# Zhiyu014/GNN-UDS

Measured on AMD Instinct MI355X. Metric: graph-steps/sec (forward rollout), |V|=10k |E|=12k d=64, higher is better.
Workload: dtype f32 storage/accumulate, GEMM operands as bf16 hi+lo split (3 MFMA products)

## Files before the change

gnn_uds_amd/csrc/kernels_fused_ws.hpp:

```cpp
#pragma once
#include "kernels_fused.hpp"

namespace uds {

constexpr int WS_NY = 4, WS_NX = FUSED_WAVES - WS_NY;
constexpr int WS_XPRIO = 1;
constexpr int WS_OCT_WD = 4;
constexpr int WS_OCT_GRP = 1;

inline int64_t fused_ws_lds_bytes(int p_cap, int q_cap, int meta_cap) {
  return 4 * ((int64_t)meta_cap + 4 * p_cap + 3 * FUSED_D + FUSED_H + 2 * (int64_t)q_cap * SEC_STRIDE + 2 * (int64_t)p_cap * FUSED_D);
}

template <int IMM>
__device__ __forceinline__ void ws_gld16(f32x4 &dst, const float *base, unsigned voff) {
  asm volatile("global_load_dwordx4 %0, %1, %2 offset:%3" : "=v"(dst) : "v"(voff), "s"(base), "n"(IMM) : "memory");
}
__device__ __forceinline__ void ws_pin4(f32x4 &a0, f32x4 &a1, f32x4 &a2, f32x4 &a3) {
  asm volatile("" : "+v"(a0), "+v"(a1), "+v"(a2), "+v"(a3));
}
__device__ __forceinline__ void row8_max4(const float (&in)[4], float (&out)[4]) {
  asm("s_nop 1\n\t" UDS_DPP4_FIRST("v_max_f32_dpp", "quad_perm:[1,0,3,2]") UDS_DPP4("v_max_f32_dpp", "quad_perm:[2,3,0,1]")
      UDS_DPP4("v_max_f32_dpp", "row_half_mirror")
      : "=&v"(out[0]), "=&v"(out[1]), "=&v"(out[2]), "=&v"(out[3])
      : "v"(in[0]), "v"(in[1]), "v"(in[2]), "v"(in[3]));
}
__device__ __forceinline__ void row8_sum4(const float (&in)[4], float (&out)[4]) {
  asm("s_nop 1\n\t" UDS_DPP4_FIRST("v_add_f32_dpp", "quad_perm:[1,0,3,2]") UDS_DPP4("v_add_f32_dpp", "quad_perm:[2,3,0,1]")
      UDS_DPP4("v_add_f32_dpp", "row_half_mirror")
      : "=&v"(out[0]), "=&v"(out[1]), "=&v"(out[2]), "=&v"(out[3])
      : "v"(in[0]), "v"(in[1]), "v"(in[2]), "v"(in[3]));
}
template <int HI>
__device__ __forceinline__ unsigned ws_add_half(unsigned pk, unsigned base) {
  unsigned r;
  if (HI) asm("v_add_u32_sdwa %0, %1, %2 dst_sel:DWORD dst_unused:UNUSED_PAD src0_sel:WORD_1 src1_sel:DWORD" : "=v"(r) : "v"(pk), "v"(base));
  else asm("v_add_u32_sdwa %0, %1, %2 dst_sel:DWORD dst_unused:UNUSED_PAD src0_sel:WORD_0 src1_sel:DWORD" : "=v"(r) : "v"(pk), "v"(base));
  return r;
}
__device__ __forceinline__ void ws_vmcnt(int n) {
  switch (n) {
    case 0: asm volatile("s_waitcnt vmcnt(0)" ::: "memory"); break;
    case 1: asm volatile("s_waitcnt vmcnt(1)" ::: "memory"); break;
    case 2: asm volatile("s_waitcnt vmcnt(2)" ::: "memory"); break;
    case 3: asm volatile("s_waitcnt vmcnt(3)" ::: "memory"); break;
    case 4: asm volatile("s_waitcnt vmcnt(4)" ::: "memory"); break;
    case 5: asm volatile("s_waitcnt vmcnt(5)" ::: "memory"); break;
    case 6: asm volatile("s_waitcnt vmcnt(6)" ::: "memory"); break;
    case 7: asm volatile("s_waitcnt vmcnt(7)" ::: "memory"); break;
    default: asm volatile("s_waitcnt vmcnt(8)" ::: "memory"); break;
  }
}

template <int ACT>
__global__ __launch_bounds__(FUSED_WAVES * 64, 2) void k_fused_ws(FusedArgs a) {
  constexpr int NT = FUSED_WAVES * 64, NY = WS_NY, NX = WS_NX;
  constexpr int FP = 64, FS = 64;
  constexpr int U = FUSED_U;
  extern __shared__ __attribute__((aligned(16))) int32_t smem[];

  const int tid = threadIdx.x, lane = tid & 63;
  const int wave = __builtin_amdgcn_readfirstlane(tid >> 6);
  const bool team_y = wave < NY;
  const int yw = wave, xw = wave - NY;

  const int W = gridDim.x, b = blockIdx.x;
  const int q8 = W / 8, r8 = W % 8, xcd = b % 8;
  const int w = (xcd < r8 ? xcd * (q8 + 1) : r8 * (q8 + 1) + (xcd - r8) * q8) + b / 8;
  const int tile = w % a.n_tiles;
  const int chunk_id = w / a.n_tiles;
  const int s_begin = chunk_id * a.chunk;
  const int s_end = min(a.S, (chunk_id + 1) * a.chunk);
  const int sd = __builtin_amdgcn_readfirstlane(a.hdr[tile * TILE_HDR_INTS + 6]);
  if (!((a.side_mask >> sd) & 1)) return;
  const FusedSide &S_ = a.side[sd];

  float *s_self = reinterpret_cast<float *>(smem + a.meta_cap);
  float *s_nbr = s_self + 2 * a.p_cap;
  float *attn = s_nbr + 2 * a.p_cap;
  float *sec = attn + 3 * FUSED_D + FUSED_H;
  float *hx = sec + 2 * a.q_cap * SEC_STRIDE;
  const int sec_buf = a.q_cap * SEC_STRIDE, hx_buf = a.p_cap * FUSED_D;

  {
    const uint4 *src = reinterpret_cast<const uint4 *>(a.blocks + (int64_t)tile * a.meta_cap);
    uint4 *dst = reinterpret_cast<uint4 *>(smem);
    for (int i = tid; i < a.meta_cap / 4; i += NT) dst[i] = src[i];
  }
  if (tid < FUSED_D) {
    attn[tid] = S_.a_self[tid] * 1.44269504088896340736f;
    attn[FUSED_D + tid] = S_.a_nbr[tid] * 1.44269504088896340736f;
    if (tid < FUSED_H) attn[2 * FUSED_D + tid] = S_.b_small ? S_.b_small[tid] : 0.f;
    attn[2 * FUSED_D + FUSED_H + tid] = S_.b_out ? S_.b_out[tid] : 0.f;
  }
  __syncthreads();
  const int n_own = __builtin_amdgcn_readfirstlane(smem[0]), n_prim = __builtin_amdgcn_readfirstlane(smem[1]),
            n_sec = __builtin_amdgcn_readfirstlane(smem[2]), flags = __builtin_amdgcn_readfirstlane(smem[3]),
            n_ovf = __builtin_amdgcn_readfirstlane(smem[4]), n_adj = __builtin_amdgcn_readfirstlane(smem[5]),
            inc_width = __builtin_amdgcn_readfirstlane(smem[7]);
  const EllOffsets off = ell_offsets(n_own, n_prim, n_sec, flags, n_ovf, n_adj);
  const int32_t *prim_ids = smem + off.prim;
  const int32_t *sec_ids = smem + off.sec;
  const uint32_t *inc_loc = reinterpret_cast<const uint32_t *>(smem + off.inc_loc);
  int32_t *inc_w = smem + off.inc_w;
  const f32x4 *inc_val4 = reinterpret_cast<const f32x4 *>(inc_w);
  const unsigned char *adj_b = reinterpret_cast<const unsigned char *>(smem + off.adj);
  const int32_t *ovf_ptr = smem + off.ovf_ptr, *ovf_loc = smem + off.ovf_loc;
  int32_t *ovf_w = smem + off.ovf_w;
  const int32_t *adj_ptr = smem + off.adj_ptr, *adj_loc = smem + off.adj_loc;

  for (int i = tid; i < ELL_INC * n_prim; i += NT) {
    const int k = inc_w[i];
    reinterpret_cast<float *>(inc_w)[i] = k >= 0 ? S_.ne_val[k] : 0.f;
  }
  if (flags & ELL_FLAG_INC_OVF)
    for (int i = tid; i < n_ovf; i += NT) reinterpret_cast<float *>(ovf_w)[i] = S_.ne_val[ovf_w[i]];
  const float *ovf_val = reinterpret_cast<const float *>(ovf_w);

#ifdef UDS_PHASE_TIMING
  unsigned long long tm_[8] = {0, 0, 0, 0, 0, 0, 0, 0}, tl_ = clock64();
  const unsigned long long rt0_ = __builtin_amdgcn_s_memrealtime(), mt0_ = tl_;
#define WS_STAMP(k) do { const unsigned long long n_ = clock64(); tm_[k] += n_ - tl_; tl_ = n_; } while (0)
#define WS_DUMP() do { if (a.dbg && lane == 0) { unsigned long long *o = a.dbg + ((size_t)blockIdx.x * 8 + wave) * 16; \
    for (int q_ = 0; q_ < 7; ++q_) o[q_] = tm_[q_]; o[12] = wave; \
    o[15] = ((__builtin_amdgcn_s_memrealtime() - rt0_) << 32) | ((clock64() - mt0_) & 0xffffffffull); \
    o[7] = 1ull | ((unsigned long long)sd << 8) | ((unsigned long long)n_own << 16) | ((unsigned long long)n_prim << 32) | ((unsigned long long)n_sec << 48); } } while (0)
#else
#define WS_STAMP(k) do { } while (0)
#define WS_DUMP() do { } while (0)
#endif
  const int64_t sec_stride = (int64_t)S_.n_sec_glob * FS, prim_stride = (int64_t)S_.n_prim_glob * FP;
  const int n_snap = s_end - s_begin;

  __syncthreads();
  if (team_y) {
    typedef float f32x16 __attribute__((ext_vector_type(16)));
    constexpr int KT32 = (FP + FUSED_H) / 16, KX32 = FP / 16, MB32 = FUSED_D / 32;
    static_assert(NY == 4, "one 32-row block per Y wave: four waves cover p_cap = 128");
    const int n32 = lane & 31, hf = lane >> 5;
    bf16x8 wh[KT32][MB32], wl[KT32][MB32];
#pragma unroll
    for (int t = 0; t < KT32; ++t)
#pragma unroll
      for (int m = 0; m < MB32; ++m) {
        wh[t][m] = __builtin_bit_cast(bf16x8, S_.w_big32[((t * MB32 + m) * 2 + 0) * 64 + lane]);
        wl[t][m] = __builtin_bit_cast(bf16x8, S_.w_big32[((t * MB32 + m) * 2 + 1) * 64 + lane]);
      }
    const int lrow = 32 * yw + n32;
    const bool valid = lrow < n_prim;
    const int lr = min(lrow, n_prim - 1);
    const unsigned prow = (unsigned)prim_ids[lr] * FP + 8u * hf;
    f32x4 pp[2 * KX32];
    const bool has_rem = S_.rem != nullptr;
    const unsigned rrow = (unsigned)prim_ids[lr] * FUSED_H + 8u * hf;
    f32x4 rm[4] = {f32x4{0.f, 0.f, 0.f, 0.f}, f32x4{0.f, 0.f, 0.f, 0.f}, f32x4{0.f, 0.f, 0.f, 0.f}, f32x4{0.f, 0.f, 0.f, 0.f}};
    const int64_t rem_stride = (int64_t)S_.n_prim_glob * FUSED_H;
    const unsigned ag_locs = inc_loc[lr];
    const f32x4 ag_vals = inc_val4[lr];
    __builtin_amdgcn_s_waitcnt(0x0F70);
    if (n_snap > 0) {
      const float *base = S_.prim_in + s_begin * prim_stride;
      static_for<2 * KX32>([&](auto i_) {
        constexpr int i = decltype(i_)::value;
        pp[i] = *reinterpret_cast<const f32x4 *>(base + prow + 16 * (i >> 1) + 4 * (i & 1));
      });
      if (has_rem) {
        const float *rb = S_.rem + s_begin * rem_stride + rrow;
        rm[0] = *reinterpret_cast<const f32x4 *>(rb);
        rm[1] = *reinterpret_cast<const f32x4 *>(rb + 4);
        rm[2] = *reinterpret_cast<const f32x4 *>(rb + 16);
        rm[3] = *reinterpret_cast<const f32x4 *>(rb + 20);
      }
    }
    WS_STAMP(0);
    lds_barrier();

    auto mfma3_32 = [&](const bf16x8 &a_h, const bf16x8 &a_l, const bf16x8 &d_h, const bf16x8 &d_l, f32x16 acc) __attribute__((always_inline)) {
      acc = __builtin_amdgcn_mfma_f32_32x32x16_bf16(a_h, d_l, acc, 0, 0, 0);
      acc = __builtin_amdgcn_mfma_f32_32x32x16_bf16(a_l, d_h, acc, 0, 0, 0);
      acc = __builtin_amdgcn_mfma_f32_32x32x16_bf16(a_h, d_h, acc, 0, 0, 0);
      return acc;
    };
    for (int k = 0; k <= n_snap; ++k) {
      if (k < n_snap && 32 * yw < n_prim) {
        const bool more = k + 1 < n_snap;
        const float *next = S_.prim_in + (s_begin + k + 1) * prim_stride;
        const float *secr = sec + (k & 1) * sec_buf;
        float *hxw = hx + (k & 1) * hx_buf;
        float *ssw = s_self + (k & 1) * a.p_cap, *snw = s_nbr + (k & 1) * a.p_cap;
        bf16x8 dh[KT32], dl[KT32];
        static_for<KX32>([&](auto t_) {
          constexpr int t = decltype(t_)::value;
          const f32x4 u0 = pp[2 * t], u1 = pp[2 * t + 1];
          split8(make_float4(u0[0], u0[1], u0[2], u0[3]), make_float4(u1[0], u1[1], u1[2], u1[3]), dh[t], dl[t]);
        });
        if (more)
          static_for<2 * KX32>([&](auto i_) {
            constexpr int i = decltype(i_)::value;
            pp[i] = *reinterpret_cast<const f32x4 *>(next + prow + 16 * (i >> 1) + 4 * (i & 1));
          });
        f32x16 acc[MB32];
#pragma unroll
        for (int m = 0; m < MB32; ++m)
#pragma unroll
          for (int r = 0; r < 16; ++r) acc[m][r] = 0.f;
#pragma unroll
        for (int t = 0; t < KX32; ++t)
#pragma unroll
          for (int m = 0; m < MB32; ++m) acc[m] = mfma3_32(wh[t][m], wl[t][m], dh[t], dl[t], acc[m]);
        float4 g0 = make_float4(rm[0][0], rm[0][1], rm[0][2], rm[0][3]), g1 = make_float4(rm[1][0], rm[1][1], rm[1][2], rm[1][3]),
               g2 = make_float4(rm[2][0], rm[2][1], rm[2][2], rm[2][3]), g3 = make_float4(rm[3][0], rm[3][1], rm[3][2], rm[3][3]);
        if (more && has_rem) {
          const float *rb = S_.rem + (s_begin + k + 1) * rem_stride + rrow;
          rm[0] = *reinterpret_cast<const f32x4 *>(rb);
          rm[1] = *reinterpret_cast<const f32x4 *>(rb + 4);
          rm[2] = *reinterpret_cast<const f32x4 *>(rb + 16);
          rm[3] = *reinterpret_cast<const f32x4 *>(rb + 20);
        }
        auto fma4 = [&](float4 &g, float wv, const float4 &u) { g.x = fmaf(wv, u.x, g.x); g.y = fmaf(wv, u.y, g.y); g.z = fmaf(wv, u.z, g.z); g.w = fmaf(wv, u.w, g.w); };
        auto add_row = [&](unsigned la, float wa) {
          const float *ra = secr + la * SEC_STRIDE + 8 * hf;
          const float4 u0 = *reinterpret_cast<const float4 *>(ra), u1 = *reinterpret_cast<const float4 *>(ra + 4);
          const float4 u2 = *reinterpret_cast<const float4 *>(ra + 16), u3 = *reinterpret_cast<const float4 *>(ra + 20);
          fma4(g0, wa, u0); fma4(g1, wa, u1); fma4(g2, wa, u2); fma4(g3, wa, u3);
        };
        add_row(ag_locs & 0xffu, ag_vals[0]);
        add_row((ag_locs >> 8) & 0xffu, ag_vals[1]);
        if (inc_width > 2) {
          add_row((ag_locs >> 16) & 0xffu, ag_vals[2]);
          add_row(ag_locs >> 24, ag_vals[3]);
        }
        if (flags & ELL_FLAG_INC_OVF)
          for (int p = ovf_ptr[lr]; p < ovf_ptr[lr + 1]; ++p) add_row((unsigned)ovf_loc[p], ovf_val[p]);
        split8(g0, g1, dh[KX32], dl[KX32]);
        split8(g2, g3, dh[KX32 + 1], dl[KX32 + 1]);
#pragma unroll
        for (int t = KX32; t < KT32; ++t)
#pragma unroll
          for (int m = 0; m < MB32; ++m) acc[m] = mfma3_32(wh[t][m], wl[t][m], dh[t], dl[t], acc[m]);
        float ps = 0.f, pn = 0.f;
#pragma unroll
        for (int m = 0; m < MB32; ++m)
#pragma unroll
          for (int gq = 0; gq < 4; ++gq) {
            const f32x4 as4 = *reinterpret_cast<const f32x4 *>(attn + 32 * m + 8 * gq + 4 * hf);
            const f32x4 an4 = *reinterpret_cast<const f32x4 *>(attn + FUSED_D + 32 * m + 8 * gq + 4 * hf);
#pragma unroll
            for (int q = 0; q < 4; ++q) {
              ps = fmaf(acc[m][4 * gq + q], as4[q], ps);
              pn = fmaf(acc[m][4 * gq + q], an4[q], pn);
            }
          }
        ps += __shfl_xor(ps, 32);
        pn += __shfl_xor(pn, 32);
        if (valid) {
          if (hf == 0) {
            ssw[lrow] = ps;
            snw[lrow] = pn;
          }
#pragma unroll
          for (int m = 0; m < MB32; ++m)
#pragma unroll
            for (int gq = 0; gq < 4; ++gq) {
              const f32x4 o = {acc[m][4 * gq], acc[m][4 * gq + 1], acc[m][4 * gq + 2], acc[m][4 * gq + 3]};
              *reinterpret_cast<f32x4 *>(hxw + lrow * FUSED_D + (((8 * m + 2 * gq + hf) ^ (lrow & 7)) << 2)) = o;
            }
        }
      }
      WS_STAMP(1);
      lds_barrier();
      WS_STAMP(2);
    }
    WS_DUMP();
  } else {
    __builtin_amdgcn_s_setprio(WS_XPRIO);
    typedef float f32x16 __attribute__((ext_vector_type(16)));
    constexpr int KS32 = FS / 16, SJ32 = (8 + NX - 1) / NX;
    const int n32 = lane & 31, hf = lane >> 5;
    bf16x8 w1h[KS32], w1l[KS32];
#pragma unroll
    for (int t = 0; t < KS32; ++t) {
      w1h[t] = __builtin_bit_cast(bf16x8, S_.w_small32[(t * 2 + 0) * 64 + lane]);
      w1l[t] = __builtin_bit_cast(bf16x8, S_.w_small32[(t * 2 + 1) * 64 + lane]);
    }
    unsigned srow[SJ32];
#pragma unroll
    for (int j = 0; j < SJ32; ++j) srow[j] = ((unsigned)sec_ids[min((xw + NX * j) * 32 + n32, n_sec - 1)] * FS + 8u * hf) * 4u;
    f32x4 sp[SJ32][2 * KS32];
    auto load_sec_at = [&](const float *base) __attribute__((always_inline)) {
      static_for<SJ32>([&](auto j_) {
        constexpr int j = decltype(j_)::value;
        ws_gld16<0>(sp[j][0], base, srow[j]);
        ws_gld16<16>(sp[j][1], base, srow[j]);
        ws_gld16<64>(sp[j][2], base, srow[j]);
        ws_gld16<80>(sp[j][3], base, srow[j]);
        ws_gld16<128>(sp[j][4], base, srow[j]);
        ws_gld16<144>(sp[j][5], base, srow[j]);
        ws_gld16<192>(sp[j][6], base, srow[j]);
        ws_gld16<208>(sp[j][7], base, srow[j]);
      });
    };
    auto load_sec = [&](int s) __attribute__((always_inline)) { load_sec_at(S_.sec_in + s * sec_stride); };
    const int ro = lane >> 3, c8 = lane & 7, hf8 = ro & 1;
    int p3_dmax[U];
    unsigned p3_pk[U][4];
    unsigned p3_jb4 = 0;
    int n_st = 0;
#pragma unroll
    for (int u = 0; u < U; ++u) {
      const int i = 8 * (NX * u + xw) + ro;
      const int ic = min(i, n_own - 1);
      int dmx;
      if (flags & ELL_FLAG_LONG_ROWS) {
        dmx = i < n_own ? adj_ptr[ic + 1] - adj_ptr[ic] : 0;
      } else {
        const unsigned long long m0 = __ballot(i < n_own && adj_b[ic * ELL_ADJ + c8] != 0xFF);
        const unsigned long long m1 = __ballot(i < n_own && adj_b[ic * ELL_ADJ + 8 + c8] != 0xFF);
        dmx = __builtin_popcountll((m0 >> (8 * ro)) & 0xffull) + __builtin_popcountll((m1 >> (8 * ro)) & 0xffull);
      }
#pragma unroll
      for (int o = 8; o < 64; o <<= 1) dmx = max(dmx, __shfl_xor(dmx, o));
      p3_dmax[u] = __builtin_amdgcn_readfirstlane(dmx);
#pragma unroll
      for (int k2 = 0; k2 < 4; ++k2) {
        unsigned pk = 0;
#pragma unroll
        for (int h = 0; h < 2; ++h) {
          const unsigned jb = adj_b[ic * ELL_ADJ + 2 * k2 + h];
          const unsigned j = (i < n_own && jb != 0xFFu) ? jb : 0u;
          pk |= (j * (FUSED_D * 4) + (((j & 7) ^ c8) << 4)) << (16 * h);
        }
        p3_pk[u][k2] = pk;
      }
      p3_jb4 |= (i < n_own ? (unsigned)adj_b[i * ELL_ADJ + c8] : 0xFFu) << (8 * u);
      if (8 * (NX * u + xw) < n_own) n_st += 2;
    }
    const float *bias_l = attn + 2 * FUSED_D + FUSED_H + 4 * c8;
    __builtin_amdgcn_s_waitcnt(0x0F70);

    auto phase1 = [&](int buf) __attribute__((always_inline)) {
      float *secw = sec + buf * sec_buf;
      static_for<SJ32>([&](auto j_) {
        constexpr int j = decltype(j_)::value;
        const int blk = xw + NX * j;
        if (blk * 32 < n_sec) {
          f32x16 acc;
#pragma unroll
          for (int gq = 0; gq < 4; ++gq) {
            const f32x4 b4 = *reinterpret_cast<const f32x4 *>(attn + 2 * FUSED_D + 8 * gq + 4 * hf);
#pragma unroll
            for (int q = 0; q < 4; ++q) acc[4 * gq + q] = b4[q];
          }
          static_for<KS32>([&](auto t_) {
            constexpr int t = decltype(t_)::value;
            const f32x4 u0 = sp[j][2 * t], u1 = sp[j][2 * t + 1];
            bf16x8 dh, dl;
            split8(make_float4(u0[0], u0[1], u0[2], u0[3]), make_float4(u1[0], u1[1], u1[2], u1[3]), dh, dl);
            acc = __builtin_amdgcn_mfma_f32_32x32x16_bf16(w1h[t], dl, acc, 0, 0, 0);
            acc = __builtin_amdgcn_mfma_f32_32x32x16_bf16(w1l[t], dh, acc, 0, 0, 0);
            acc = __builtin_amdgcn_mfma_f32_32x32x16_bf16(w1h[t], dh, acc, 0, 0, 0);
          });
          const int lrow = blk * 32 + n32;
          if (lrow < n_sec) {
#pragma unroll
            for (int gq = 0; gq < 4; ++gq) {
              f32x4 o;
#pragma unroll
              for (int q = 0; q < 4; ++q) o[q] = fused_act<ACT>(acc[4 * gq + q], a.act);
              *reinterpret_cast<f32x4 *>(secw + lrow * SEC_STRIDE + 8 * gq + 4 * hf) = o;
            }
          }
        }
      });
    };
    auto pin_rows = [&]() __attribute__((always_inline)) {
      static_for<SJ32>([&](auto j_) {
        constexpr int j = decltype(j_)::value;
        ws_pin4(sp[j][0], sp[j][1], sp[j][2], sp[j][3]);
        ws_pin4(sp[j][4], sp[j][5], sp[j][6], sp[j][7]);
      });
    };

    if (n_snap > 0) {
      load_sec(s_begin);
      ws_vmcnt(0);
      pin_rows();
      phase1(0);
      if (n_snap > 1) load_sec(s_begin + 1);
    }
    WS_STAMP(0);
    lds_barrier();

    auto phase3o = [&](float *out_snap, int buf) __attribute__((always_inline)) {
      const float *hxr = hx + buf * hx_buf;
      const float *ssr = s_self + buf * a.p_cap, *snr = s_nbr + buf * a.p_cap;
      int d0 = p3_dmax[0], d1 = p3_dmax[1], d2 = p3_dmax[2], d3 = p3_dmax[3];
      asm volatile("" : "+s"(d0), "+s"(d1), "+s"(d2), "+s"(d3));
      const int e3 = d3, e2 = max(e3, d2), e1 = max(e2, d1), e0 = max(e1, d0);
      if (e0 == 0) return;

      float ss[U], lg0[U], lg1[U], w0[U], w1[U], den[U];
      bool ok[U], has0[U], has1[U];
      unsigned jb0[U], jb1[U];
      int joff1[U];
#pragma unroll
      for (int u = 0; u < U; ++u) {
        ok[u] = 8 * (NX * u + xw) + ro < n_own;
        jb0[u] = (p3_jb4 >> (8 * u)) & 0xFFu;
        ss[u] = ssr[8 * (NX * u + xw) + ro];
      }
#pragma unroll
      for (int u = 0; u < U; ++u) has0[u] = ok[u] && jb0[u] != 0xFFu;
      f32x4 acc0[U], acc1[U];
#pragma unroll
      for (int u = 0; u < U; ++u) acc0[u] = acc1[u] = f32x4{0.f, 0.f, 0.f, 0.f};
      if (e0 <= 16) {
        const bool ext = e0 > 8;
        float sn[U];
#pragma unroll
        for (int u = 0; u < U; ++u) sn[u] = snr[jb0[u]];
        asm volatile("" : "+v"(sn[0]), "+v"(sn[1]), "+v"(sn[2]), "+v"(sn[3]));
#pragma unroll
        for (int u = 0; u < U; ++u) {
          const float sv = ss[u] + sn[u];
          lg0[u] = has0[u] ? fmaxf(sv, 0.2f * sv) : -INFINITY;
        }
        float mx[U];
        row8_max4(lg0, mx);
        if (ext) {
          float m1[U];
#pragma unroll
          for (int u = 0; u < U; ++u) jb1[u] = adj_b[(8 * (NX * u + xw) + ro) * ELL_ADJ + 8 + c8];
          asm volatile("" : "+v"(jb1[0]), "+v"(jb1[1]), "+v"(jb1[2]), "+v"(jb1[3]));
#pragma unroll
          for (int u = 0; u < U; ++u) sn[u] = snr[jb1[u]];
          asm volatile("" : "+v"(sn[0]), "+v"(sn[1]), "+v"(sn[2]), "+v"(sn[3]));
#pragma unroll
          for (int u = 0; u < U; ++u) {
            has1[u] = ok[u] && jb1[u] != 0xFFu;
            const int j1 = has1[u] ? (int)jb1[u] : 0;
            joff1[u] = j1 * (FUSED_D * 4) + ((j1 & 7) << 4);
            const float sv = ss[u] + sn[u];
            lg1[u] = has1[u] ? fmaxf(sv, 0.2f * sv) : -INFINITY;
          }
          row8_max4(lg1, m1);
#pragma unroll
          for (int u = 0; u < U; ++u) mx[u] = fmaxf(mx[u], m1[u]);
        }
#pragma unroll
        for (int u = 0; u < U; ++u) w0[u] = has0[u] ? __builtin_amdgcn_exp2f(lg0[u] - mx[u]) : 0.f;
        row8_sum4(w0, den);
        if (ext) {
          float d1s[U];
#pragma unroll
          for (int u = 0; u < U; ++u) w1[u] = has1[u] ? __builtin_amdgcn_exp2f(lg1[u] - mx[u]) : 0.f;
          row8_sum4(w1, d1s);
#pragma unroll
          for (int u = 0; u < U; ++u) den[u] += d1s[u];
        }
        typedef const __attribute__((address_space(3))) f32x4 *lds_f4;
        const unsigned hxa0 = lds_addr(hxr) + 128 * hf8, hxa1 = lds_addr(hxr) + 128 - 128 * hf8;
        const int cx = c8 << 4;
        const int bp = (lane & 56) << 2;
        using I1 = std::integral_constant<int, 1>; using I2 = std::integral_constant<int, 2>;
        using I3 = std::integral_constant<int, 3>; using I4 = std::integral_constant<int, 4>;
        auto step = [&](auto SET_, auto K_, auto A_) __attribute__((always_inline)) {
          constexpr int SET = decltype(SET_)::value, K = decltype(K_)::value, A = decltype(A_)::value,
                        Wd = (8 - K < WS_OCT_WD ? 8 - K : WS_OCT_WD);
          constexpr int G = WS_OCT_GRP;
          static_for<(A + G - 1) / G>([&](auto g_) {
            constexpr int u0 = decltype(g_)::value * G, GA = (A - u0 < G ? A - u0 : G);
            f32x4 h0[GA][Wd], h1[GA][Wd];
            static_for<GA>([&](auto u_) {
              constexpr int ul = decltype(u_)::value, u = u0 + ul;
              static_for<Wd>([&](auto i_) {
                constexpr int i = decltype(i_)::value, k = K + i;
                unsigned ad = 0;
                if (SET) ad = (unsigned)__builtin_amdgcn_ds_bpermute(bp + 4 * k, joff1[u]) ^ cx;
                unsigned ad0, ad1;
                if (SET) {
                  ad0 = ad + hxa0;
                  ad1 = ad + hxa1;
                } else {
                  ad0 = ws_add_half<k & 1>(p3_pk[u][k >> 1], hxa0);
                  ad1 = ws_add_half<k & 1>(p3_pk[u][k >> 1], hxa1);
                }
                h0[ul][i] = *(lds_f4)(uintptr_t)ad0;
                h1[ul][i] = *(lds_f4)(uintptr_t)ad1;
              });
            });
            static_for<GA>([&](auto u_) {
              constexpr int ul = decltype(u_)::value, u = u0 + ul;
              static_for<Wd>([&](auto i_) {
                constexpr int i = decltype(i_)::value, k = K + i;
                float wv;
                if (SET) wv = __int_as_float(__builtin_amdgcn_ds_bpermute(bp + 4 * k, __float_as_int(w1[u])));
                else {
                  const int wi = __float_as_int(w0[u]);
                  int t = __builtin_amdgcn_update_dpp(wi, wi, 0x150 + k, 0xf, 0xf, true);
                  t = __builtin_amdgcn_update_dpp(t, wi, 0x150 + 8 + k, 0xf, 0xc, false);
                  wv = __int_as_float(t);
                }
#pragma unroll
                for (int q = 0; q < 4; ++q) {
                  acc0[u][q] = fmaf(wv, h0[ul][i][q], acc0[u][q]);
                  acc1[u][q] = fmaf(wv, h1[ul][i][q], acc1[u][q]);
                }
              });
            });
          });
        };
        static_for<(8 + WS_OCT_WD - 1) / WS_OCT_WD>([&](auto t_) {
          constexpr int K = decltype(t_)::value * WS_OCT_WD;
          using IK = std::integral_constant<int, K>;
          using S0 = std::integral_constant<int, 0>;
          if (K < e3) step(S0{}, IK{}, I4{});
          else if (K < e2) step(S0{}, IK{}, I3{});
          else if (K < e1) step(S0{}, IK{}, I2{});
          else if (K < e0) step(S0{}, IK{}, I1{});
        });
        if (ext)
          static_for<(8 + WS_OCT_WD - 1) / WS_OCT_WD>([&](auto t_) {
            constexpr int K = decltype(t_)::value * WS_OCT_WD;
            using IK = std::integral_constant<int, K>;
            using S1 = std::integral_constant<int, 1>;
            if (K + 8 < e3) step(S1{}, IK{}, I4{});
            else if (K + 8 < e2) step(S1{}, IK{}, I3{});
            else if (K + 8 < e1) step(S1{}, IK{}, I2{});
            else if (K + 8 < e0) step(S1{}, IK{}, I1{});
          });
      } else {
#pragma unroll
        for (int u = 0; u < U; ++u) {
          const int i = 8 * (NX * u + xw) + ro;
          const int b0 = i < n_own ? adj_ptr[i] : 0;
          const int dg = i < n_own ? adj_ptr[i + 1] - b0 : 0;
          float mx = -INFINITY;
          for (int p = b0; p < b0 + dg; ++p) mx = fmaxf(mx, leaky02(ss[u] + snr[adj_loc[p]]));
          den[u] = 0.f;
          for (int p = b0; p < b0 + dg; ++p) {
            const int jj = adj_loc[p];
            const float wv = __builtin_amdgcn_exp2f(leaky02(ss[u] + snr[jj]) - mx);
            const f32x4 v0 = *reinterpret_cast<const f32x4 *>(hxr + jj * FUSED_D + 32 * hf8 + ((c8 ^ (jj & 7)) << 2));
            const f32x4 v1 = *reinterpret_cast<const f32x4 *>(hxr + jj * FUSED_D + 32 - 32 * hf8 + ((c8 ^ (jj & 7)) << 2));
            den[u] += wv;
#pragma unroll
            for (int q = 0; q < 4; ++q) {
              acc0[u][q] = fmaf(wv, v0[q], acc0[u][q]);
              acc1[u][q] = fmaf(wv, v1[q], acc1[u][q]);
            }
          }
        }
      }
      f32x4 bo0 = *reinterpret_cast<const f32x4 *>(bias_l + 32 * hf8), bo1 = *reinterpret_cast<const f32x4 *>(bias_l + 32 - 32 * hf8);
      int pid[U];
#pragma unroll
      for (int u = 0; u < U; ++u) pid[u] = prim_ids[8 * (NX * u + xw) + ro];
      asm volatile("" : "+v"(pid[0]), "+v"(pid[1]), "+v"(pid[2]), "+v"(pid[3]), "+v"(bo0), "+v"(bo1));
      float *out_s = out_snap + (4 * c8 + 32 * hf8);
      const int o1_off = 32 - 64 * hf8;
#pragma unroll
      for (int u = 0; u < U; ++u) {
        if (ok[u]) {
          const float inv = __builtin_amdgcn_rcpf(den[u]);
          f32x4 o0, o1;
#pragma unroll
          for (int q = 0; q < 4; ++q) {
            o0[q] = fused_act<ACT>(fmaf(acc0[u][q], inv, bo0[q]), a.act);
            o1[q] = fused_act<ACT>(fmaf(acc1[u][q], inv, bo1[q]), a.act);
          }
          float *orow = out_s + (int64_t)pid[u] * FUSED_D;
          *reinterpret_cast<f32x4 *>(orow) = o0;
          *reinterpret_cast<f32x4 *>(orow + o1_off) = o1;
        }
      }
    };
    const float *sec_next = S_.sec_in + (int64_t)(s_begin + 2) * sec_stride;
    float *out_next = S_.out + (int64_t)s_begin * S_.n_prim_glob * FUSED_D;
    const int64_t out_stride = (int64_t)S_.n_prim_glob * FUSED_D;
    for (int k = 0; k <= n_snap; ++k) {
      if (k + 1 < n_snap) {
        ws_vmcnt(k >= 2 ? n_st : 0);
        pin_rows();
        phase1((k + 1) & 1);
        if (k + 2 < n_snap) load_sec_at(sec_next);
        sec_next += sec_stride;
      }
      WS_STAMP(3);
      if (k >= 1) {
        phase3o(out_next, (k - 1) & 1);
        out_next += out_stride;
        WS_STAMP(4);
      }
      WS_STAMP(1);
      lds_barrier();
      WS_STAMP(2);
    }
    WS_DUMP();
  }
}

}
```

Baseline: 292,300.

## Overlap tile metadata staging and ne_val gather with weight and input loads

Reads tile header fields straight from global memory so the ELL offsets are known before the metadata block is copied into LDS. The block copy, attention-vector loads and ne_val gather are split into issue and land steps, so their latency overlaps with the weight-register loads and the first sec/prim input loads. Prim and sec row ids also come from global, which drops a block-wide barrier at kernel start. In exchange there are more redundant global reads and more ordering assumptions between LDS writes and the later barriers. There is also a new static assumption that one gather element per thread covers ELL_INC*n_prim.

```diff
diff --git a/gnn_uds_amd/csrc/kernels_fused_ws.hpp b/gnn_uds_amd/csrc/kernels_fused_ws.hpp
--- a/gnn_uds_amd/csrc/kernels_fused_ws.hpp
+++ b/gnn_uds_amd/csrc/kernels_fused_ws.hpp
@@ -71,9 +71,19 @@
   const int chunk_id = w / a.n_tiles;
   const int s_begin = chunk_id * a.chunk;
   const int s_end = min(a.S, (chunk_id + 1) * a.chunk);
+#ifdef UDS_PHASE_TIMING
+  unsigned long long tm_[8] = {0, 0, 0, 0, 0, 0, 0, 0}, tl_ = clock64();
+  const unsigned long long rt0_ = __builtin_amdgcn_s_memrealtime(), mt0_ = tl_;
+#endif
+  const int32_t *gblk = a.blocks + (int64_t)tile * a.meta_cap;
   const int sd = __builtin_amdgcn_readfirstlane(a.hdr[tile * TILE_HDR_INTS + 6]);
+  int hd_[TILE_HDR_INTS];
+#pragma unroll
+  for (int q = 0; q < TILE_HDR_INTS; ++q) hd_[q] = __builtin_amdgcn_readfirstlane(gblk[q]);
   if (!((a.side_mask >> sd) & 1)) return;
   const FusedSide &S_ = a.side[sd];
+  const int n_own = hd_[0], n_prim = hd_[1], n_sec = hd_[2], flags = hd_[3], n_ovf = hd_[4], n_adj = hd_[5], inc_width = hd_[7];
+  const EllOffsets off = ell_offsets(n_own, n_prim, n_sec, flags, n_ovf, n_adj);
 
   float *s_self = reinterpret_cast<float *>(smem + a.meta_cap);
   float *s_nbr = s_self + 2 * a.p_cap;
@@ -82,25 +92,7 @@
   float *hx = sec + 2 * a.q_cap * SEC_STRIDE;
   const int sec_buf = a.q_cap * SEC_STRIDE, hx_buf = a.p_cap * FUSED_D;
 
-  {
-    const uint4 *src = reinterpret_cast<const uint4 *>(a.blocks + (int64_t)tile * a.meta_cap);
-    uint4 *dst = reinterpret_cast<uint4 *>(smem);
-    for (int i = tid; i < a.meta_cap / 4; i += NT) dst[i] = src[i];
-  }
-  if (tid < FUSED_D) {
-    attn[tid] = S_.a_self[tid] * 1.44269504088896340736f;
-    attn[FUSED_D + tid] = S_.a_nbr[tid] * 1.44269504088896340736f;
-    if (tid < FUSED_H) attn[2 * FUSED_D + tid] = S_.b_small ? S_.b_small[tid] : 0.f;
-    attn[2 * FUSED_D + FUSED_H + tid] = S_.b_out ? S_.b_out[tid] : 0.f;
-  }
-  __syncthreads();
-  const int n_own = __builtin_amdgcn_readfirstlane(smem[0]), n_prim = __builtin_amdgcn_readfirstlane(smem[1]),
-            n_sec = __builtin_amdgcn_readfirstlane(smem[2]), flags = __builtin_amdgcn_readfirstlane(smem[3]),
-            n_ovf = __builtin_amdgcn_readfirstlane(smem[4]), n_adj = __builtin_amdgcn_readfirstlane(smem[5]),
-            inc_width = __builtin_amdgcn_readfirstlane(smem[7]);
-  const EllOffsets off = ell_offsets(n_own, n_prim, n_sec, flags, n_ovf, n_adj);
   const int32_t *prim_ids = smem + off.prim;
-  const int32_t *sec_ids = smem + off.sec;
   const uint32_t *inc_loc = reinterpret_cast<const uint32_t *>(smem + off.inc_loc);
   int32_t *inc_w = smem + off.inc_w;
   const f32x4 *inc_val4 = reinterpret_cast<const f32x4 *>(inc_w);
@@ -108,18 +100,53 @@
   const int32_t *ovf_ptr = smem + off.ovf_ptr, *ovf_loc = smem + off.ovf_loc;
   int32_t *ovf_w = smem + off.ovf_w;
   const int32_t *adj_ptr = smem + off.adj_ptr, *adj_loc = smem + off.adj_loc;
-
-  for (int i = tid; i < ELL_INC * n_prim; i += NT) {
-    const int k = inc_w[i];
-    reinterpret_cast<float *>(inc_w)[i] = k >= 0 ? S_.ne_val[k] : 0.f;
-  }
-  if (flags & ELL_FLAG_INC_OVF)
-    for (int i = tid; i < n_ovf; i += NT) reinterpret_cast<float *>(ovf_w)[i] = S_.ne_val[ovf_w[i]];
   const float *ovf_val = reinterpret_cast<const float *>(ovf_w);
 
+  const int n4 = a.meta_cap / 4;
+  const uint4 *blk4 = reinterpret_cast<const uint4 *>(gblk);
+  uint4 blk0;
+  float at_s = 0.f, at_n = 0.f, at_bs = 0.f, at_bo = 0.f;
+  auto issue_block = [&]() __attribute__((always_inline)) {
+    blk0 = blk4[min(tid, n4 - 1)];
+    if (wave == 0) {
+      at_s = S_.a_self[lane];
+      at_n = S_.a_nbr[lane];
+      if (lane < FUSED_H && S_.b_small) at_bs = S_.b_small[lane];
+      if (S_.b_out) at_bo = S_.b_out[lane];
+    }
+  };
+  auto block_to_lds = [&]() __attribute__((always_inline)) {
+    asm volatile("" ::: "memory");
+    uint4 *dst = reinterpret_cast<uint4 *>(smem);
+    if (tid < n4) dst[tid] = blk0;
+    for (int i = tid + NT; i < n4; i += NT) dst[i] = blk4[i];
+    if (wave == 0) {
+      attn[lane] = at_s * 1.44269504088896340736f;
+      attn[FUSED_D + lane] = at_n * 1.44269504088896340736f;
+      if (lane < FUSED_H) attn[2 * FUSED_D + lane] = at_bs;
+      attn[2 * FUSED_D + FUSED_H + lane] = at_bo;
+    }
+    __syncthreads();
+  };
+  static_assert(ELL_INC * 32 * NY <= NT, "one gather element per thread covers the rows the Y team multiplies");
+  const int n_inc = ELL_INC * n_prim;
+  float ne_v = 0.f, ov_v = 0.f;
+  auto gather_issue = [&]() __attribute__((always_inline)) {
+    if (tid < n_inc) {
+      const int k = inc_w[tid];
+      if (k >= 0) ne_v = S_.ne_val[k];
+    }
+    if ((flags & ELL_FLAG_INC_OVF) && tid < n_ovf) ov_v = S_.ne_val[ovf_w[tid]];
+  };
+  auto gather_land = [&]() __attribute__((always_inline)) {
+    if (tid < n_inc) reinterpret_cast<float *>(inc_w)[tid] = ne_v;
+    if (flags & ELL_FLAG_INC_OVF) {
+      if (tid < n_ovf) reinterpret_cast<float *>(ovf_w)[tid] = ov_v;
+      for (int i = tid + NT; i < n_ovf; i += NT) reinterpret_cast<float *>(ovf_w)[i] = S_.ne_val[ovf_w[i]];
+    }
+  };
+
 #ifdef UDS_PHASE_TIMING
-  unsigned long long tm_[8] = {0, 0, 0, 0, 0, 0, 0, 0}, tl_ = clock64();
-  const unsigned long long rt0_ = __builtin_amdgcn_s_memrealtime(), mt0_ = tl_;
 #define WS_STAMP(k) do { const unsigned long long n_ = clock64(); tm_[k] += n_ - tl_; tl_ = n_; } while (0)
 #define WS_DUMP() do { if (a.dbg && lane == 0) { unsigned long long *o = a.dbg + ((size_t)blockIdx.x * 8 + wave) * 16; \
     for (int q_ = 0; q_ < 7; ++q_) o[q_] = tm_[q_]; o[12] = wave; \
@@ -132,12 +159,16 @@
   const int64_t sec_stride = (int64_t)S_.n_sec_glob * FS, prim_stride = (int64_t)S_.n_prim_glob * FP;
   const int n_snap = s_end - s_begin;
 
-  __syncthreads();
   if (team_y) {
     typedef float f32x16 __attribute__((ext_vector_type(16)));
     constexpr int KT32 = (FP + FUSED_H) / 16, KX32 = FP / 16, MB32 = FUSED_D / 32;
     static_assert(NY == 4, "one 32-row block per Y wave: four waves cover p_cap = 128");
     const int n32 = lane & 31, hf = lane >> 5;
+    const int lrow = 32 * yw + n32;
+    const bool valid = lrow < n_prim;
+    const int lr = min(lrow, n_prim - 1);
+    issue_block();
+    const int prim_id = gblk[off.prim + lr];
     bf16x8 wh[KT32][MB32], wl[KT32][MB32];
 #pragma unroll
     for (int t = 0; t < KT32; ++t)
@@ -146,18 +177,13 @@
         wh[t][m] = __builtin_bit_cast(bf16x8, S_.w_big32[((t * MB32 + m) * 2 + 0) * 64 + lane]);
         wl[t][m] = __builtin_bit_cast(bf16x8, S_.w_big32[((t * MB32 + m) * 2 + 1) * 64 + lane]);
       }
-    const int lrow = 32 * yw + n32;
-    const bool valid = lrow < n_prim;
-    const int lr = min(lrow, n_prim - 1);
-    const unsigned prow = (unsigned)prim_ids[lr] * FP + 8u * hf;
+    block_to_lds();
+    const unsigned prow = (unsigned)prim_id * FP + 8u * hf;
     f32x4 pp[2 * KX32];
     const bool has_rem = S_.rem != nullptr;
-    const unsigned rrow = (unsigned)prim_ids[lr] * FUSED_H + 8u * hf;
+    const unsigned rrow = (unsigned)prim_id * FUSED_H + 8u * hf;
     f32x4 rm[4] = {f32x4{0.f, 0.f, 0.f, 0.f}, f32x4{0.f, 0.f, 0.f, 0.f}, f32x4{0.f, 0.f, 0.f, 0.f}, f32x4{0.f, 0.f, 0.f, 0.f}};
     const int64_t rem_stride = (int64_t)S_.n_prim_glob * FUSED_H;
-    const unsigned ag_locs = inc_loc[lr];
-    const f32x4 ag_vals = inc_val4[lr];
-    __builtin_amdgcn_s_waitcnt(0x0F70);
     if (n_snap > 0) {
       const float *base = S_.prim_in + s_begin * prim_stride;
       static_for<2 * KX32>([&](auto i_) {
@@ -172,8 +198,13 @@
         rm[3] = *reinterpret_cast<const f32x4 *>(rb + 20);
       }
     }
+    gather_issue();
+    const unsigned ag_locs = inc_loc[lr];
+    gather_land();
+    __builtin_amdgcn_s_waitcnt(0x0F70);
     WS_STAMP(0);
     lds_barrier();
+    const f32x4 ag_vals = inc_val4[lr];
 
     auto mfma3_32 = [&](const bf16x8 &a_h, const bf16x8 &a_l, const bf16x8 &d_h, const bf16x8 &d_l, f32x16 acc) __attribute__((always_inline)) {
       acc = __builtin_amdgcn_mfma_f32_32x32x16_bf16(a_h, d_l, acc, 0, 0, 0);
@@ -277,15 +308,20 @@
     typedef float f32x16 __attribute__((ext_vector_type(16)));
     constexpr int KS32 = FS / 16, SJ32 = (8 + NX - 1) / NX;
     const int n32 = lane & 31, hf = lane >> 5;
+    issue_block();
+    int sec_id[SJ32];
+#pragma unroll
+    for (int j = 0; j < SJ32; ++j) sec_id[j] = gblk[off.sec + min((xw + NX * j) * 32 + n32, n_sec - 1)];
     bf16x8 w1h[KS32], w1l[KS32];
 #pragma unroll
     for (int t = 0; t < KS32; ++t) {
       w1h[t] = __builtin_bit_cast(bf16x8, S_.w_small32[(t * 2 + 0) * 64 + lane]);
       w1l[t] = __builtin_bit_cast(bf16x8, S_.w_small32[(t * 2 + 1) * 64 + lane]);
     }
+    block_to_lds();
     unsigned srow[SJ32];
 #pragma unroll
-    for (int j = 0; j < SJ32; ++j) srow[j] = ((unsigned)sec_ids[min((xw + NX * j) * 32 + n32, n_sec - 1)] * FS + 8u * hf) * 4u;
+    for (int j = 0; j < SJ32; ++j) srow[j] = ((unsigned)sec_id[j] * FS + 8u * hf) * 4u;
     f32x4 sp[SJ32][2 * KS32];
     auto load_sec_at = [&](const float *base) __attribute__((always_inline)) {
       static_for<SJ32>([&](auto j_) {
@@ -302,6 +338,8 @@
     };
     auto load_sec = [&](int s) __attribute__((always_inline)) { load_sec_at(S_.sec_in + s * sec_stride); };
     const int ro = lane >> 3, c8 = lane & 7, hf8 = ro & 1;
+    if (n_snap > 0) load_sec(s_begin);
+    gather_issue();
     int p3_dmax[U];
     unsigned p3_pk[U][4];
     unsigned p3_jb4 = 0;
@@ -336,6 +374,7 @@
       if (8 * (NX * u + xw) < n_own) n_st += 2;
     }
     const float *bias_l = attn + 2 * FUSED_D + FUSED_H + 4 * c8;
+    gather_land();
     __builtin_amdgcn_s_waitcnt(0x0F70);
 
     auto phase1 = [&](int buf) __attribute__((always_inline)) {
@@ -382,7 +421,6 @@
     };
 
     if (n_snap > 0) {
-      load_sec(s_begin);
       ws_vmcnt(0);
       pin_rows();
       phase1(0);
```

Measured after the change: 297,900 (median of 6 runs). 1.02x the previous value.
